# filthyrake/vlog

Measured on AMD Instinct MI355X. Metric: audio-sec transcribed per wall-sec (RTFx), large-v3, 1/2/4/8 MI355X; WER delta, higher is better.
Workload: dtype bf16; 1 GPU; config 4: large-v3 bf16 greedy, timestamps on, 150 x 30 s windows per GPU of the seeded speech-like corpus (uniform transcript lengths), window-sharded; model=large-v3, windows_per_gpu=150, decoder_steps=113, decode=all-rows batch, decoder_row_steps=16950, corpus=uniform, parallelism=window-shard x1

## Files before the change

vlog_amd/csrc/attn_enc.hip:

```cpp
#include "common.h"
#include <cstdlib>
#include <stdexcept>
#include <string>
#include <type_traits>

#define HD 64
#define KT 64
#define VT_LD 68

__device__ __forceinline__ int kswz(int row, int ch) { return row * HD + ((ch ^ ((row >> 1) & 7)) << 3); }

__global__ __launch_bounds__(256) void attn_enc_kernel(const bf16* __restrict__ qkv, bf16* __restrict__ out, int T,
                                                       int d, float scale_log2) {
  __shared__ __attribute__((aligned(16))) bf16 sK[KT * HD];
  __shared__ __attribute__((aligned(16))) bf16 sVt[HD * VT_LD];
  const int tid = threadIdx.x, lane = tid & 63, wv = tid >> 6;
  const int g = lane >> 4, ql = lane & 15;
  const int h = blockIdx.y, b = blockIdx.z;
  const long long ld = 3LL * d;
  const bf16* base = qkv + (long long)b * T * ld;
  const int q0 = blockIdx.x * 64 + wv * 16;

  bf16x8 qf[2];
  {
    const int q = q0 + ql;
#pragma unroll
    for (int kk = 0; kk < 2; ++kk) {
      if (q < T) qf[kk] = *(const bf16x8*)(base + (long long)q * ld + h * HD + kk * 32 + 8 * g);
      else qf[kk] = bf16x8{};
    }
  }

  f32x4 o[4];
#pragma unroll
  for (int i = 0; i < 4; ++i) o[i] = f32x4{0.f, 0.f, 0.f, 0.f};
  float m_run = -INFINITY, l_run = 0.f;

  i32x4 rk[2], rv[2];
  const int nt = (T + KT - 1) / KT;
#define LOAD_TILE(t_)                                                                       \
  {                                                                                         \
    _Pragma("unroll") for (int i = 0; i < 2; ++i) {                                         \
      const int c = tid + i * 256, key = (t_) * KT + (c >> 3), ch = c & 7;                  \
      if (key < T) {                                                                        \
        const bf16* p = base + (long long)key * ld + h * HD + ch * 8;                        \
        rk[i] = *(const i32x4*)(p + d);                                                     \
        rv[i] = *(const i32x4*)(p + 2 * d);                                                 \
      } else {                                                                              \
        rk[i] = i32x4{0, 0, 0, 0};                                                          \
        rv[i] = i32x4{0, 0, 0, 0};                                                          \
      }                                                                                     \
    }                                                                                       \
  }
  LOAD_TILE(0);
  for (int t = 0; t < nt; ++t) {
    __syncthreads();
#pragma unroll
    for (int i = 0; i < 2; ++i) {
      const int c = tid + i * 256, key = c >> 3, ch = c & 7;
      *(i32x4*)(&sK[kswz(key, ch)]) = rk[i];
      bf16x8 vv = __builtin_bit_cast(bf16x8, rv[i]);
#pragma unroll
      for (int e = 0; e < 8; ++e) sVt[(ch * 8 + e) * VT_LD + key] = vv[e];
    }
    __syncthreads();
    if (t + 1 < nt) LOAD_TILE(t + 1);

    f32x4 s[4];
#pragma unroll
    for (int mi = 0; mi < 4; ++mi) {
      s[mi] = f32x4{0.f, 0.f, 0.f, 0.f};
#pragma unroll
      for (int kk = 0; kk < 2; ++kk) {
        const bf16x8 ka = *(const bf16x8*)(&sK[kswz(mi * 16 + ql, kk * 4 + g)]);
        s[mi] = __builtin_amdgcn_mfma_f32_16x16x32_bf16(ka, qf[kk], s[mi], 0, 0, 0);
      }
    }
    float tmax = -INFINITY;
    const int kbase = t * KT;
#pragma unroll
    for (int mi = 0; mi < 4; ++mi)
#pragma unroll
      for (int e = 0; e < 4; ++e) {
        const int key = kbase + mi * 16 + 4 * g + e;
        float v = s[mi][e] * scale_log2;
        if (key >= T) v = -INFINITY;
        s[mi][e] = v;
        tmax = fmaxf(tmax, v);
      }
    tmax = fmaxf(tmax, __shfl_xor(tmax, 16, 64));
    tmax = fmaxf(tmax, __shfl_xor(tmax, 32, 64));
    const float m_new = fmaxf(m_run, tmax);
    const float alpha = exp2f(m_run - m_new);
    float psum = 0.f;
#pragma unroll
    for (int mi = 0; mi < 4; ++mi)
#pragma unroll
      for (int e = 0; e < 4; ++e) {
        const float p = exp2f(s[mi][e] - m_new);
        s[mi][e] = p;
        psum += p;
      }
    psum += __shfl_xor(psum, 16, 64);
    psum += __shfl_xor(psum, 32, 64);
    l_run = l_run * alpha + psum;
    m_run = m_new;
#pragma unroll
    for (int ni = 0; ni < 4; ++ni) o[ni] *= alpha;

#pragma unroll
    for (int ks = 0; ks < 2; ++ks) {
      bf16x8 pb;
#pragma unroll
      for (int e = 0; e < 4; ++e) {
        pb[e] = f2bf(s[2 * ks][e]);
        pb[4 + e] = f2bf(s[2 * ks + 1][e]);
      }
#pragma unroll
      for (int ni = 0; ni < 4; ++ni) {
        const bf16* vr = &sVt[(ni * 16 + ql) * VT_LD + ks * 32 + 4 * g];
        const bf16x4 lo = *(const bf16x4*)(vr);
        const bf16x4 hi = *(const bf16x4*)(vr + 16);
        bf16x8 va;
#pragma unroll
        for (int e = 0; e < 4; ++e) { va[e] = lo[e]; va[4 + e] = hi[e]; }
        o[ni] = __builtin_amdgcn_mfma_f32_16x16x32_bf16(va, pb, o[ni], 0, 0, 0);
      }
    }
  }
#undef LOAD_TILE

  const int q = q0 + ql;
  if (q < T) {
    const float inv = 1.0f / l_run;
    bf16* orow = out + ((long long)b * T + q) * d + h * HD;
#pragma unroll
    for (int ni = 0; ni < 4; ++ni) {
      bf16x4 w;
#pragma unroll
      for (int e = 0; e < 4; ++e) w[e] = f2bf(o[ni][e] * inv);
      *(bf16x4*)(orow + ni * 16 + 4 * g) = w;
    }
  }
}

#define A2_KT 64
#define A2_THR 8.0f
typedef __attribute__((ext_vector_type(4))) short i16x4;
typedef __attribute__((ext_vector_type(2))) int i32x2;

__device__ __forceinline__ int a2_kslot(int r, int c) { return r * 64 + ((c ^ ((r >> 1) & 7)) << 3); }
__device__ __forceinline__ int a2_vslot(int r, int c) { return r * 64 + ((c ^ (((r >> 1) & 1) << 2)) << 3); }

__global__ __launch_bounds__(256, 2) void attn_enc_v2_kernel(const bf16* __restrict__ qkv, bf16* __restrict__ out,
                                                             int T, int d, float scale_log2, int n_head) {
  __shared__ __attribute__((aligned(16))) bf16 smem[2 * 2 * A2_KT * HD];
  const int tid = threadIdx.x, lane = tid & 63, wv = tid >> 6;
  const int ql = lane & 31, hh = lane >> 5;
  const int nqt = (T + 127) / 128;
  int qt, h, b;
  {
    const int nwg = gridDim.x, bid = blockIdx.x, xcd = bid & 7, q8 = nwg >> 3, r8 = nwg & 7;
    const int wgid = (xcd < r8 ? xcd * (q8 + 1) : r8 * (q8 + 1) + (xcd - r8) * q8) + (bid >> 3);
    qt = wgid % nqt;
    const int rest = wgid / nqt;
    h = rest % n_head;
    b = rest / n_head;
  }
  const long long ld = 3LL * d;
  const bf16* base = qkv + (long long)b * T * ld + h * HD;
  const int q = qt * 128 + wv * 32 + ql;

  bf16x8 qf[4];
  {
    const int qc = min(q, T - 1);
#pragma unroll
    for (int s = 0; s < 4; ++s) {
      const bf16x8 v = *(const bf16x8*)(base + (long long)qc * ld + 16 * s + 8 * hh);
#pragma unroll
      for (int j = 0; j < 8; ++j) qf[s][j] = f2bf(bf2f(v[j]) * scale_log2);
    }
  }
  f32x16 o[2];
#pragma unroll
  for (int i = 0; i < 2; ++i)
#pragma unroll
    for (int r = 0; r < 16; ++r) o[i][r] = 0.f;
  float m_run = -INFINITY, l_run = 0.f;

  i32x4 rk[2], rv[2];
  const int nt = (T + A2_KT - 1) / A2_KT;
  auto load_tile = [&](int t) {
#pragma unroll
    for (int i = 0; i < 2; ++i) {
      const int c = tid + i * 256, key = min(t * A2_KT + (c >> 3), T - 1), ch = c & 7;
      const bf16* p = base + (long long)key * ld + ch * 8;
      rk[i] = *(const i32x4*)(p + d);
      rv[i] = *(const i32x4*)(p + 2 * d);
    }
  };
  auto store_tile = [&](int buf) {
    bf16* sK = smem + buf * (2 * A2_KT * HD);
    bf16* sV = sK + A2_KT * HD;
#pragma unroll
    for (int i = 0; i < 2; ++i) {
      const int c = tid + i * 256, r = c >> 3, ch = c & 7;
      *(i32x4*)(sK + a2_kslot(r, ch)) = rk[i];
      *(i32x4*)(sV + a2_vslot(r, ch)) = rv[i];
    }
  };
  load_tile(0);
  store_tile(0);
  __syncthreads();

  const int G = lane >> 4, gi = lane & 15, gq = gi >> 2, gp = gi & 3;
  for (int t = 0; t < nt; ++t) {
    const bf16* sK = smem + (t & 1) * (2 * A2_KT * HD);
    const bf16* sV = sK + A2_KT * HD;
    if (t + 1 < nt) load_tile(t + 1);

    f32x16 sc[2];
#pragma unroll
    for (int kb = 0; kb < 2; ++kb) {
#pragma unroll
      for (int r = 0; r < 16; ++r) sc[kb][r] = 0.f;
#pragma unroll
      for (int s = 0; s < 4; ++s) {
        const bf16x8 ka = *(const bf16x8*)(sK + a2_kslot(kb * 32 + ql, 2 * s + hh));
        sc[kb] = __builtin_amdgcn_mfma_f32_32x32x16_bf16(ka, qf[s], sc[kb], 0, 0, 0);
      }
    }
    if (t == nt - 1) {
#pragma unroll
      for (int kb = 0; kb < 2; ++kb)
#pragma unroll
        for (int r = 0; r < 16; ++r) {
          const int key = t * A2_KT + kb * 32 + 8 * (r >> 2) + 4 * hh + (r & 3);
          if (key >= T) sc[kb][r] = -INFINITY;
        }
    }
    float mx = sc[0][0];
#pragma unroll
    for (int kb = 0; kb < 2; ++kb)
#pragma unroll
      for (int r = 0; r < 16; ++r) mx = fmaxf(mx, sc[kb][r]);
    mx = fmaxf(mx, __shfl_xor(mx, 32, 64));
    if (__any(mx > m_run + A2_THR)) {
      const float mn = fmaxf(m_run, mx);
      const float alpha = __builtin_amdgcn_exp2f(m_run - mn);
      l_run *= alpha;
#pragma unroll
      for (int i = 0; i < 2; ++i)
#pragma unroll
        for (int r = 0; r < 16; ++r) o[i][r] *= alpha;
      m_run = mn;
    }
    bf16x8 pf[2][2];
#pragma unroll
    for (int kb = 0; kb < 2; ++kb)
#pragma unroll
      for (int r = 0; r < 16; ++r) {
        const float pv = __builtin_amdgcn_exp2f(sc[kb][r] - m_run);
        l_run += pv;
        pf[kb][r >> 3][r & 7] = f2bf(pv);
      }
#pragma unroll
    for (int kb = 0; kb < 2; ++kb)
#pragma unroll
      for (int s = 0; s < 2; ++s)
#pragma unroll
        for (int hb = 0; hb < 2; ++hb) {
          bf16x8 va;
#ifndef A2_SCALAR_V
          i32x2 vw[2];
#endif
#pragma unroll
          for (int jh = 0; jh < 2; ++jh) {
            const int row = kb * 32 + 16 * s + 8 * jh + 4 * (G >> 1) + gq;
            const int col = 32 * hb + 16 * (G & 1) + 4 * gp;
#ifdef A2_SCALAR_V
            const int rowb = row - gq, hdc = 32 * hb + 16 * (G & 1) + gi;
#pragma unroll
            for (int e = 0; e < 4; ++e) va[4 * jh + e] = sV[a2_vslot(rowb + e, hdc >> 3) + (hdc & 7)];
#else
            const bf16* ad = sV + a2_vslot(row, col >> 3) + (col & 7);
            vw[jh] = __builtin_bit_cast(i32x2, __builtin_amdgcn_ds_read_tr16_b64_v4i16(
                                                   (__attribute__((address_space(3))) i16x4*)(ad)));
#endif
          }
#ifndef A2_SCALAR_V
          va = __builtin_bit_cast(bf16x8, i32x4{vw[0][0], vw[0][1], vw[1][0], vw[1][1]});
#endif
          o[hb] = __builtin_amdgcn_mfma_f32_32x32x16_bf16(va, pf[kb][s], o[hb], 0, 0, 0);
        }
    if (t + 1 < nt) store_tile((t + 1) & 1);
    __syncthreads();
  }

  l_run += __shfl_xor(l_run, 32, 64);
  if (q < T) {
    const float inv = 1.0f / l_run;
    bf16* orow = out + ((long long)b * T + q) * d + h * HD;
#pragma unroll
    for (int hb = 0; hb < 2; ++hb)
#pragma unroll
      for (int g = 0; g < 4; ++g) {
        bf16x4 w;
#pragma unroll
        for (int e = 0; e < 4; ++e) w[e] = f2bf(o[hb][4 * g + e] * inv);
        *(bf16x4*)(orow + 32 * hb + 8 * g + 4 * hh) = w;
      }
  }
}

__device__ __forceinline__ void a3_scores(const bf16* sK, const bf16x8 (&qf)[4], int ql, int hh, f32x16 (&sc)[2]) {
#pragma unroll
  for (int kb = 0; kb < 2; ++kb)
#pragma unroll
    for (int r = 0; r < 16; ++r) sc[kb][r] = 0.f;
#pragma unroll
  for (int s = 0; s < 4; ++s)
#pragma unroll
    for (int kb = 0; kb < 2; ++kb) {
      const bf16x8 ka = *(const bf16x8*)(sK + a2_kslot(kb * 32 + ql, 2 * s + hh));
      sc[kb] = __builtin_amdgcn_mfma_f32_32x32x16_bf16(ka, qf[s], sc[kb], 0, 0, 0);
    }
}

__global__ __launch_bounds__(256, 2) void attn_enc_v3_kernel(const bf16* __restrict__ qkv, bf16* __restrict__ out,
                                                             int T, int d, float scale_log2, int n_head) {
  __shared__ __attribute__((aligned(16))) bf16 smem[3 * 2 * A2_KT * HD];
  const int tid = threadIdx.x, lane = tid & 63, wv = tid >> 6;
  const int ql = lane & 31, hh = lane >> 5;
  const int nqt = (T + 127) / 128;
  int qt, h, b;
  {
    const int nwg = gridDim.x, bid = blockIdx.x, xcd = bid & 7, q8 = nwg >> 3, r8 = nwg & 7;
    const int wgid = (xcd < r8 ? xcd * (q8 + 1) : r8 * (q8 + 1) + (xcd - r8) * q8) + (bid >> 3);
    qt = wgid % nqt;
    const int rest = wgid / nqt;
    h = rest % n_head;
    b = rest / n_head;
  }
  const long long ld = 3LL * d;
  const bf16* base = qkv + (long long)b * T * ld + h * HD;
  const int q = qt * 128 + wv * 32 + ql;

  bf16x8 qf[4];
  {
    const int qc = min(q, T - 1);
#pragma unroll
    for (int s = 0; s < 4; ++s) {
      const bf16x8 v = *(const bf16x8*)(base + (long long)qc * ld + 16 * s + 8 * hh);
#pragma unroll
      for (int j = 0; j < 8; ++j) qf[s][j] = f2bf(bf2f(v[j]) * scale_log2);
    }
  }
  f32x16 o[2];
#pragma unroll
  for (int i = 0; i < 2; ++i)
#pragma unroll
    for (int r = 0; r < 16; ++r) o[i][r] = 0.f;
  float m_run = -INFINITY, l_run = 0.f;

  i32x4 rk[2], rv[2];
  const int nt = (T + A2_KT - 1) / A2_KT;
  auto load_tile = [&](int t) {
#pragma unroll
    for (int i = 0; i < 2; ++i) {
      const int c = tid + i * 256, key = min(t * A2_KT + (c >> 3), T - 1), ch = c & 7;
      const bf16* p = base + (long long)key * ld + ch * 8;
      rk[i] = *(const i32x4*)(p + d);
      rv[i] = *(const i32x4*)(p + 2 * d);
    }
  };
  auto store_tile = [&](int slot) {
    bf16* sK = smem + slot * (2 * A2_KT * HD);
    bf16* sV = sK + A2_KT * HD;
#pragma unroll
    for (int i = 0; i < 2; ++i) {
      const int c = tid + i * 256, r = c >> 3, ch = c & 7;
      *(i32x4*)(sK + a2_kslot(r, ch)) = rk[i];
      *(i32x4*)(sV + a2_vslot(r, ch)) = rv[i];
    }
  };
  load_tile(0);
  store_tile(0);
  if (nt > 1) {
    load_tile(1);
    store_tile(1);
  }
  __syncthreads();

  const int G = lane >> 4, gi = lane & 15, gq = gi >> 2, gp = gi & 3;
  f32x16 sc[2];
  a3_scores(smem, qf, ql, hh, sc);

  auto tile = [&](int t, int slot, auto last_tag) {
    constexpr bool LAST = decltype(last_tag)::value;
    const bf16* sV = smem + slot * (2 * A2_KT * HD) + A2_KT * HD;
    f32x16 sn[2];
    if constexpr (!LAST) load_tile(t + 2);
    if constexpr (LAST) {
#pragma unroll
      for (int kb = 0; kb < 2; ++kb)
#pragma unroll
        for (int r = 0; r < 16; ++r) {
          const int key = t * A2_KT + kb * 32 + 8 * (r >> 2) + 4 * hh + (r & 3);
          if (key >= T) sc[kb][r] = -INFINITY;
        }
    }
    float mx = sc[0][0];
#pragma unroll
    for (int kb = 0; kb < 2; ++kb)
#pragma unroll
      for (int r = 0; r < 16; ++r) mx = fmaxf(mx, sc[kb][r]);
    mx = fmaxf(mx, __shfl_xor(mx, 32, 64));
    if (__any(mx > m_run + A2_THR)) {
      const float mn = fmaxf(m_run, mx);
      const float alpha = __builtin_amdgcn_exp2f(m_run - mn);
      l_run *= alpha;
#pragma unroll
      for (int i = 0; i < 2; ++i)
#pragma unroll
        for (int r = 0; r < 16; ++r) o[i][r] *= alpha;
      m_run = mn;
    }
    if constexpr (!LAST) a3_scores(smem + (slot == 2 ? 0 : slot + 1) * (2 * A2_KT * HD), qf, ql, hh, sn);
    bf16x8 pf[2][2];
#pragma unroll
    for (int kb = 0; kb < 2; ++kb)
#pragma unroll
      for (int r = 0; r < 16; ++r) {
        const float pv = __builtin_amdgcn_exp2f(sc[kb][r] - m_run);
        l_run += pv;
        pf[kb][r >> 3][r & 7] = f2bf(pv);
      }
#pragma unroll
    for (int kb = 0; kb < 2; ++kb)
#pragma unroll
      for (int s = 0; s < 2; ++s)
#pragma unroll
        for (int hb = 0; hb < 2; ++hb) {
          i32x2 vw[2];
#pragma unroll
          for (int jh = 0; jh < 2; ++jh) {
            const int row = kb * 32 + 16 * s + 8 * jh + 4 * (G >> 1) + gq;
            const int col = 32 * hb + 16 * (G & 1) + 4 * gp;
            const bf16* ad = sV + a2_vslot(row, col >> 3) + (col & 7);
            vw[jh] = __builtin_bit_cast(i32x2, __builtin_amdgcn_ds_read_tr16_b64_v4i16(
                                                   (__attribute__((address_space(3))) i16x4*)(ad)));
          }
          const bf16x8 va = __builtin_bit_cast(bf16x8, i32x4{vw[0][0], vw[0][1], vw[1][0], vw[1][1]});
          o[hb] = __builtin_amdgcn_mfma_f32_32x32x16_bf16(va, pf[kb][s], o[hb], 0, 0, 0);
        }
    if constexpr (!LAST) {
      store_tile(slot == 0 ? 2 : slot - 1);
      __syncthreads();
#pragma unroll
      for (int kb = 0; kb < 2; ++kb) sc[kb] = sn[kb];
    }
  };
  int slot = 0;
  for (int t = 0; t < nt - 1; ++t) {
    tile(t, slot, std::false_type{});
    slot = slot == 2 ? 0 : slot + 1;
  }
  tile(nt - 1, slot, std::true_type{});

  l_run += __shfl_xor(l_run, 32, 64);
  if (q < T) {
    const float inv = 1.0f / l_run;
    bf16* orow = out + ((long long)b * T + q) * d + h * HD;
#pragma unroll
    for (int hb = 0; hb < 2; ++hb)
#pragma unroll
      for (int g = 0; g < 4; ++g) {
        bf16x4 w;
#pragma unroll
        for (int e = 0; e < 4; ++e) w[e] = f2bf(o[hb][4 * g + e] * inv);
        *(bf16x4*)(orow + 32 * hb + 8 * g + 4 * hh) = w;
      }
  }
}

static int attn_enc_form() {
  static const int v = [] {
    const char* e1 = std::getenv("VLOG_AMD_ATTN_V1");
    if (e1 && e1[0] == '1') return 1;
    const char* e = std::getenv("VLOG_AMD_ATTN_V");
    const int f = e ? std::atoi(e) : 2;
    return (f >= 1 && f <= 3) ? f : 2;
  }();
  return v;
}

void launch_attn_enc(const bf16* qkv, bf16* out, int B, int T, int d, int n_head, hipStream_t st) {
  if (B <= 0) return;
  if (d != n_head * HD) throw std::runtime_error("attn_enc: head_dim must be 64");
  const float scale_log2 = 0.125f * 1.4426950408889634f;
  const int form = attn_enc_form();
  if (form == 1) {
    dim3 grid((T + 63) / 64, n_head, B);
    hipLaunchKernelGGL(attn_enc_kernel, grid, dim3(256), 0, st, qkv, out, T, d, scale_log2);
  } else {
    const long long nblk = (long long)((T + 127) / 128) * n_head * B;
    if (nblk > (1LL << 31) - 1) throw std::runtime_error("attn_enc: grid too large");
    if (form == 3)
      hipLaunchKernelGGL(attn_enc_v3_kernel, dim3((unsigned)nblk), dim3(256), 0, st, qkv, out, T, d, scale_log2, n_head);
    else
      hipLaunchKernelGGL(attn_enc_v2_kernel, dim3((unsigned)nblk), dim3(256), 0, st, qkv, out, T, d, scale_log2, n_head);
  }
  WM_LAUNCH_CHECK("attn_enc_kernel");
}
```

Before: 3938 audio_s/s.

## Add v4 encoder attention kernel with XCD-aware block mapping and hoisted softmax max

```diff
diff --git a/vlog_amd/csrc/attn_enc.hip b/vlog_amd/csrc/attn_enc.hip
--- a/vlog_amd/csrc/attn_enc.hip
+++ b/vlog_amd/csrc/attn_enc.hip
@@ -484,15 +484,246 @@
   }
 }
 
+template <bool NEGM, bool HOIST, bool LMAX>
+__global__ __launch_bounds__(256, 2) void attn_enc_v4_kernel(const bf16* __restrict__ qkv, bf16* __restrict__ out,
+                                                             int T, int d, float scale_log2, int n_head) {
+  __shared__ __attribute__((aligned(16))) bf16 smem[2 * 2 * A2_KT * HD];
+  const int tid = threadIdx.x, lane = tid & 63, wv = tid >> 6;
+  const int ql = lane & 31, hh = lane >> 5;
+  const int nqt = (T + 127) / 128;
+  int qt, h, b;
+  {
+    const int nwg = gridDim.x, bid = blockIdx.x, xcd = bid & 7, q8 = nwg >> 3, r8 = nwg & 7;
+    const int wgid = (xcd < r8 ? xcd * (q8 + 1) : r8 * (q8 + 1) + (xcd - r8) * q8) + (bid >> 3);
+    qt = wgid % nqt;
+    const int rest = wgid / nqt;
+    h = rest % n_head;
+    b = rest / n_head;
+  }
+  const long long ld = 3LL * d;
+  const bf16* base = qkv + (long long)b * T * ld + h * HD;
+  const int q = qt * 128 + wv * 32 + ql;
+
+  bf16x8 qf[4];
+  {
+    const int qc = min(q, T - 1);
+#pragma unroll
+    for (int s = 0; s < 4; ++s) {
+      const bf16x8 v = *(const bf16x8*)(base + (long long)qc * ld + 16 * s + 8 * hh);
+#pragma unroll
+      for (int j = 0; j < 8; ++j) qf[s][j] = f2bf(bf2f(v[j]) * scale_log2);
+    }
+  }
+  f32x16 o[2], negm;
+#pragma unroll
+  for (int r = 0; r < 16; ++r) o[0][r] = o[1][r] = negm[r] = 0.f;
+  float m_run = -INFINITY, l_run = 0.f;
+
+  i32x4 rk[2], rv[2];
+  const int nt = (T + A2_KT - 1) / A2_KT;
+  auto load_tile = [&](int t) {
+#pragma unroll
+    for (int i = 0; i < 2; ++i) {
+      const int c = tid + i * 256, key = min(t * A2_KT + (c >> 3), T - 1), ch = c & 7;
+      const bf16* p = base + (long long)key * ld + ch * 8;
+      rk[i] = *(const i32x4*)(p + d);
+      rv[i] = *(const i32x4*)(p + 2 * d);
+    }
+  };
+  const unsigned voff = (unsigned)(((tid >> 3) * ld + (tid & 7) * 8) * 2);
+  auto load_tile_steady = [&](int t) {
+    const char* tb = (const char*)(base + (long long)t * A2_KT * ld);
+#pragma unroll
+    for (int i = 0; i < 2; ++i) {
+      const char* rb = tb + (long long)i * 32 * ld * 2;
+      rk[i] = *(const i32x4*)(rb + (long long)d * 2 + voff);
+      rv[i] = *(const i32x4*)(rb + (long long)d * 4 + voff);
+    }
+  };
+  auto store_tile = [&](int buf) {
+    bf16* sK = smem + buf * (2 * A2_KT * HD);
+    bf16* sV = sK + A2_KT * HD;
+#pragma unroll
+    for (int i = 0; i < 2; ++i) {
+      const int c = tid + i * 256, r = c >> 3, ch = c & 7;
+      *(i32x4*)(sK + a2_kslot(r, ch)) = rk[i];
+      *(i32x4*)(sV + a2_vslot(r, ch)) = rv[i];
+    }
+  };
+  load_tile(0);
+  store_tile(0);
+  __syncthreads();
+
+  const int G = lane >> 4, gi = lane & 15, gq = gi >> 2, gp = gi & 3;
+  auto tile = [&](int t, auto first_tag, auto last_tag, auto pf_tag) {
+    constexpr bool FIRST = decltype(first_tag)::value, LAST = decltype(last_tag)::value;
+    constexpr int PF = decltype(pf_tag)::value;
+    static_assert(LAST == (PF == 0), "exactly the last tile prefetches nothing");
+    const bf16* sK = smem + (t & 1) * (2 * A2_KT * HD);
+    const bf16* sV = sK + A2_KT * HD;
+    if constexpr (PF == 1 && HOIST) load_tile_steady(t + 1);
+    else if constexpr (PF != 0) load_tile(t + 1);
+
+    f32x16 sc[2];
+#pragma unroll
+    for (int kb = 0; kb < 2; ++kb) {
+      if constexpr (NEGM && !FIRST) sc[kb] = negm;
+      else {
+#pragma unroll
+        for (int r = 0; r < 16; ++r) sc[kb][r] = 0.f;
+      }
+#pragma unroll
+      for (int s = 0; s < 4; ++s) {
+        const bf16x8 ka = *(const bf16x8*)(sK + a2_kslot(kb * 32 + ql, 2 * s + hh));
+        sc[kb] = __builtin_amdgcn_mfma_f32_32x32x16_bf16(ka, qf[s], sc[kb], 0, 0, 0);
+      }
+    }
+    if constexpr (LAST) {
+#pragma unroll
+      for (int kb = 0; kb < 2; ++kb)
+#pragma unroll
+        for (int r = 0; r < 16; ++r) {
+          const int key = t * A2_KT + kb * 32 + 8 * (r >> 2) + 4 * hh + (r & 3);
+          if (key >= T) sc[kb][r] = -INFINITY;
+        }
+    }
+    float mx = sc[0][0];
+#pragma unroll
+    for (int kb = 0; kb < 2; ++kb)
+#pragma unroll
+      for (int r = 0; r < 16; ++r) mx = fmaxf(mx, sc[kb][r]);
+    if constexpr (FIRST || !LMAX) mx = fmaxf(mx, __shfl_xor(mx, 32, 64));
+    if constexpr (FIRST) {
+      m_run = mx;
+      if constexpr (NEGM) {
+#pragma unroll
+        for (int r = 0; r < 16; ++r) negm[r] = -m_run;
+#pragma unroll
+        for (int kb = 0; kb < 2; ++kb)
+#pragma unroll
+          for (int r = 0; r < 16; ++r) sc[kb][r] -= m_run;
+      }
+    } else if constexpr (NEGM) {
+      if (__any(mx > A2_THR)) {
+        if constexpr (LMAX) mx = fmaxf(mx, __shfl_xor(mx, 32, 64));
+        const float dl = fmaxf(mx, 0.f);
+        const float alpha = __builtin_amdgcn_exp2f(-dl);
+        l_run *= alpha;
+#pragma unroll
+        for (int i = 0; i < 2; ++i)
+#pragma unroll
+          for (int r = 0; r < 16; ++r) o[i][r] *= alpha;
+        m_run += dl;
+#pragma unroll
+        for (int r = 0; r < 16; ++r) negm[r] = -m_run;
+#pragma unroll
+        for (int kb = 0; kb < 2; ++kb)
+#pragma unroll
+          for (int r = 0; r < 16; ++r) sc[kb][r] -= dl;
+      }
+    } else {
+      if (__any(mx > m_run + A2_THR)) {
+        if constexpr (LMAX) mx = fmaxf(mx, __shfl_xor(mx, 32, 64));
+        const float mn = fmaxf(m_run, mx);
+        const float alpha = __builtin_amdgcn_exp2f(m_run - mn);
+        l_run *= alpha;
+#pragma unroll
+        for (int i = 0; i < 2; ++i)
+#pragma unroll
+          for (int r = 0; r < 16; ++r) o[i][r] *= alpha;
+        m_run = mn;
+      }
+    }
+    bf16x8 pf[2][2];
+#pragma unroll
+    for (int kb = 0; kb < 2; ++kb)
+#pragma unroll
+      for (int r = 0; r < 16; ++r) {
+        float pv;
+        if constexpr (NEGM) pv = __builtin_amdgcn_exp2f(sc[kb][r]);
+        else pv = __builtin_amdgcn_exp2f(sc[kb][r] - m_run);
+        l_run += pv;
+        pf[kb][r >> 3][r & 7] = f2bf(pv);
+      }
+#pragma unroll
+    for (int kb = 0; kb < 2; ++kb)
+#pragma unroll
+      for (int s = 0; s < 2; ++s)
+#pragma unroll
+        for (int hb = 0; hb < 2; ++hb) {
+          i32x2 vw[2];
+#pragma unroll
+          for (int jh = 0; jh < 2; ++jh) {
+            const int row = kb * 32 + 16 * s + 8 * jh + 4 * (G >> 1) + gq;
+            const int col = 32 * hb + 16 * (G & 1) + 4 * gp;
+            const bf16* ad = sV + a2_vslot(row, col >> 3) + (col & 7);
+            vw[jh] = __builtin_bit_cast(i32x2, __builtin_amdgcn_ds_read_tr16_b64_v4i16(
+                                                   (__attribute__((address_space(3))) i16x4*)(ad)));
+          }
+          const bf16x8 va = __builtin_bit_cast(bf16x8, i32x4{vw[0][0], vw[0][1], vw[1][0], vw[1][1]});
+          o[hb] = __builtin_amdgcn_mfma_f32_32x32x16_bf16(va, pf[kb][s], o[hb], 0, 0, 0);
+        }
+    if constexpr (!LAST) {
+      store_tile((t + 1) & 1);
+      __syncthreads();
+    }
+  };
+  using Y = std::true_type;
+  using N = std::false_type;
+  using PF0 = std::integral_constant<int, 0>;
+  using PF1 = std::integral_constant<int, 1>;
+  using PF2 = std::integral_constant<int, 2>;
+  if (nt == 1) {
+    tile(0, Y{}, Y{}, PF0{});
+  } else {
+    if (nt == 2) tile(0, Y{}, N{}, PF2{});
+    else tile(0, Y{}, N{}, PF1{});
+    for (int t = 1; t < nt - 2; ++t) tile(t, N{}, N{}, PF1{});
+    if (nt > 2) tile(nt - 2, N{}, N{}, PF2{});
+    tile(nt - 1, N{}, Y{}, PF0{});
+  }
+
+  l_run += __shfl_xor(l_run, 32, 64);
+  if (q < T) {
+    const float inv = 1.0f / l_run;
+    bf16* orow = out + ((long long)b * T + q) * d + h * HD;
+#pragma unroll
+    for (int hb = 0; hb < 2; ++hb)
+#pragma unroll
+      for (int g = 0; g < 4; ++g) {
+        bf16x4 w;
+#pragma unroll
+        for (int e = 0; e < 4; ++e) w[e] = f2bf(o[hb][4 * g + e] * inv);
+        *(bf16x4*)(orow + 32 * hb + 8 * g + 4 * hh) = w;
+      }
+  }
+}
+
+#define A4_SW_DEFAULT 7
 static int attn_enc_form() {
   static const int v = [] {
     const char* e1 = std::getenv("VLOG_AMD_ATTN_V1");
     if (e1 && e1[0] == '1') return 1;
     const char* e = std::getenv("VLOG_AMD_ATTN_V");
-    const int f = e ? std::atoi(e) : 2;
-    return (f >= 1 && f <= 3) ? f : 2;
+    const int f = e ? std::atoi(e) : 4;
+    return (f >= 1 && f <= 4) ? f : 4;
   }();
   return v;
+}
+static int attn_enc_v4_switches() {
+  static const int v = [] {
+    const char* e = std::getenv("VLOG_AMD_ATTN_V4_SW");
+    const int f = e ? std::atoi(e) : A4_SW_DEFAULT;
+    return (f >= 0 && f <= 7) ? f : A4_SW_DEFAULT;
+  }();
+  return v;
+}
+
+template <int SW>
+static void launch_attn_enc_v4(unsigned nblk, hipStream_t st, const bf16* qkv, bf16* out, int T, int d, float scale_log2,
+                               int n_head) {
+  hipLaunchKernelGGL((attn_enc_v4_kernel<(SW & 1) != 0, (SW & 2) != 0, (SW & 4) != 0>), dim3(nblk), dim3(256), 0, st,
+                     qkv, out, T, d, scale_log2, n_head);
 }
 
 void launch_attn_enc(const bf16* qkv, bf16* out, int B, int T, int d, int n_head, hipStream_t st) {
@@ -508,8 +739,14 @@
     if (nblk > (1LL << 31) - 1) throw std::runtime_error("attn_enc: grid too large");
     if (form == 3)
       hipLaunchKernelGGL(attn_enc_v3_kernel, dim3((unsigned)nblk), dim3(256), 0, st, qkv, out, T, d, scale_log2, n_head);
-    else
+    else if (form == 2)
       hipLaunchKernelGGL(attn_enc_v2_kernel, dim3((unsigned)nblk), dim3(256), 0, st, qkv, out, T, d, scale_log2, n_head);
+    else {
+      using Fn = void (*)(unsigned, hipStream_t, const bf16*, bf16*, int, int, float, int);
+      static const Fn tab[8] = {launch_attn_enc_v4<0>, launch_attn_enc_v4<1>, launch_attn_enc_v4<2>, launch_attn_enc_v4<3>,
+                                launch_attn_enc_v4<4>, launch_attn_enc_v4<5>, launch_attn_enc_v4<6>, launch_attn_enc_v4<7>};
+      tab[attn_enc_v4_switches()]((unsigned)nblk, st, qkv, out, T, d, scale_log2, n_head);
+    }
   }
   WM_LAUNCH_CHECK("attn_enc_kernel");
 }
```

New measurement: 3951 audio_s/s (median of 6 runs). Within noise of the previous version (+0.3%).
